# megvii-research/basedet

Hardware: AMD Instinct MI355X
Metric: images/sec training RetinaNet-R50-FPN 1333x800 (higher is better)
Workload: dtype bf16; 1 GPU; retinanet_r50_800x1344 train step (fwd+bwd+allreduce+SGD), DummyLoader boxes, random-init weights, inputs resident in HBM; per_gpu_batch=16, global_batch=16, parallelism=dp1

## Files before the change

### basedet_amd/_lib.py

```python
import ctypes as C
import os

import torch

_HERE = os.path.dirname(os.path.abspath(__file__))
LIB_PATH = os.environ.get("BASEDET_HIP_LIB") or os.path.join(_HERE, "lib", "libbasedet_hip.so")

BD_MAX_SEGS = 8
ABI_VERSION = 112
EPI_RELU, EPI_ADD_BEFORE, EPI_ADD_AFTER, EPI_MASK, EPI_SPARSE = 1, 2, 4, 8, 16


class BasedetHipError(RuntimeError):
    pass


class ConvDesc(C.Structure):
    _fields_ = [
        ("N", C.c_int32), ("Cin", C.c_int32), ("Cout", C.c_int32), ("R", C.c_int32), ("S", C.c_int32),
        ("stride", C.c_int32), ("pad", C.c_int32), ("nseg", C.c_int32),
        ("Hi", C.c_int32 * BD_MAX_SEGS), ("Wi", C.c_int32 * BD_MAX_SEGS),
        ("Ho", C.c_int32 * BD_MAX_SEGS), ("Wo", C.c_int32 * BD_MAX_SEGS),
        ("in_off", C.c_int32 * BD_MAX_SEGS), ("out_off", C.c_int32 * BD_MAX_SEGS),
        ("in_pix_per_img", C.c_int32), ("out_pix_per_img", C.c_int32),
        ("route", C.c_int32 * 4), ("sr_seed", C.c_uint32),
        ("gskip", C.c_int32), ("gskip_ws", C.c_void_p), ("gskip_ws_bytes", C.c_size_t),
        ("gskip_gmap", C.c_void_p), ("gskip_gmap_bytes", C.c_size_t), ("gskip_dxmap", C.c_void_p), ("gskip_dxmap_bytes", C.c_size_t),
        ("gskip_dx_clean", C.c_int32),
        ("fwd_map", C.c_void_p), ("fwd_map_bytes", C.c_size_t), ("fwd_clean", C.c_int32),
    ]


class PackDesc(C.Structure):
    _fields_ = [("w", C.c_void_p), ("row_scale", C.c_void_p), ("w_fwd", C.c_void_p), ("w_dgrad", C.c_void_p),
                ("Cout", C.c_int32), ("RS", C.c_int32), ("Cin", C.c_int32), ("block_start", C.c_int32)]


class ImageDesc(C.Structure):
    _fields_ = [("offset", C.c_int64), ("src_h", C.c_int32), ("src_w", C.c_int32), ("dst_h", C.c_int32), ("dst_w", C.c_int32),
                ("flip", C.c_int32), ("reserved_", C.c_int32 * 1)]


_P, _I, _L, _F, _Z = C.c_void_p, C.c_int, C.c_int64, C.c_float, C.c_size_t
_D = C.POINTER(ConvDesc)
# ... 223 lines not shown
```

### basedet_amd/csrc/conv3x3_pp.hip

```cpp
#include "conv3x3_pp128_body.h"

namespace {

constexpr int PH = 4, PW = 16, IH = PH + 2, IW = PW + 2;
constexpr int NPATCH = 4;
constexpr int XROWS = NPATCH * IH * IW;
constexpr int X_PITCH = 144;
constexpr int X_BYTES = XROWS * X_PITCH;
constexpr int XPASSES = 7;
constexpr int TILE_CO = 256;
constexpr int W_SLOT = TILE_CO * 128;
constexpr int NSLOT = 3;
constexpr int W_BYTES = NSLOT * W_SLOT;
constexpr int GTAB_TILES = 16;
constexpr int GTAB_BYTES = GTAB_TILES * NPATCH * 32;
constexpr int LDS_BYTES = W_BYTES + X_BYTES + TILE_CO * 4 + GTAB_BYTES;
constexpr int MAX_SEG = BD_MAX_SEGS;
constexpr int TAIL_CO = 64;

struct PSeg { int patch_start, H, W, pw, src_off, dst_off; float inv_pw; };

struct PParams {
    const bf16_raw* src;
    const bf16_raw* w;
// ... 696 lines not shown
        const int grid128 = cdiv(p.total_patches, NPATCH) * cdiv(p.CO, 128);
        if (!gn_part && g_patch_pp < 2 && 3 * cdiv(grid, 256) >= 2 * cdiv(grid128, 256)) return 1;
    }
    BD_ONCE_PER_DEVICE(
        (void)hipFuncSetAttribute(reinterpret_cast<const void*>(&conv3x3_pp_kernel<0>), hipFuncAttributeMaxDynamicSharedMemorySize, LDS_BYTES);
        (void)hipFuncSetAttribute(reinterpret_cast<const void*>(&conv3x3_pp_kernel<1>), hipFuncAttributeMaxDynamicSharedMemorySize, LDS_BYTES);
        (void)hipFuncSetAttribute(reinterpret_cast<const void*>(&conv3x3_pp_kernel<1, false, true>), hipFuncAttributeMaxDynamicSharedMemorySize,
                                  LDS_BYTES);
        (void)hipFuncSetAttribute(reinterpret_cast<const void*>(&conv3x3_pp_kernel<0, false, true>), hipFuncAttributeMaxDynamicSharedMemorySize,
                                  LDS_BYTES));
    bd_note_kernel("conv3x3_pp_kernel");
    if (sparse) {
        const int tot = p.total_patches;
        p.sp_keep_dead = in_place ? 1 : 0;
        p.sp_stride = tot;
        if (d->gskip_gmap) {
            BdGskipMap gm;
            bd_gskip_map_layout(d, 0, &gm);
            const int* m = (const int*)d->gskip_gmap;
            p.sp_hdr = m; p.sp_live = m + gm.live; p.sp_list = m + gm.list;
        } else {
            int* mk = (int*)d->gskip_ws;
            p.sp_live = mk + tot; p.sp_list = mk + 2 * tot; p.sp_count = mk + 3 * tot;
            bd_gskip_scan(d, src, PH, PW, mk, stream);
            bd_gskip_compact(d, PH, PW, mk, mk + tot, mk + 2 * tot, mk + 3 * tot, stream);
        }
        if (d->gskip_dxmap) {
            BdGskipMap xm;
            bd_gskip_map_layout(d, 1, &xm);
            p.sp_ohdr = (int*)d->gskip_dxmap; p.sp_olist = p.sp_ohdr + xm.list;
// ... 72 lines not shown
```

### basedet_amd/csrc/conv_igemm.hip

```cpp
#include "igemm_params.h"

using namespace igemm;

namespace {

template <int BK>
struct Cfg {
    static constexpr int CHUNKS = BK / 8;
    static constexpr int ROWS_PER_PASS = 256 / CHUNKS;
    static constexpr int PASSES = 128 / ROWS_PER_PASS;
    static constexpr int LDS_STRIDE = BK == 64 ? 160 : 64;
    static constexpr int TILE_BYTES = 128 * LDS_STRIDE;
    __device__ static __forceinline__ int off(int row, int chunk) {
        if constexpr (BK == 64) return row * LDS_STRIDE + chunk * 16;
        else return row * 64 + ((chunk ^ ((row >> 1) & 3)) << 4);
    }
};

template <int BK, bool PRE, bool BUF>
__global__ __launch_bounds__(256) void conv_igemm_kernel(const IgemmParams p) {
    using C = Cfg<BK>;
    extern __shared__ __attribute__((aligned(16))) unsigned char smem[];
    unsigned char* tiles = smem;
    unsigned int* s_tapmask = reinterpret_cast<unsigned int*>(smem);
// ... 527 lines not shown
    BD_ROUTE(d);
    return conv2d_fwd_impl(d, x, w_packed, bias, add, y, ybits, y8, q_scale, flags, stream);
}

extern "C" int bd_conv2d_fwd_bits(const bd_conv_desc* d, const void* x, const void* w_packed, const float* bias, const void* add, void* y,
                                  uint32_t* ybits, int flags, bd_stream_t stream) {
    BD_ROUTE(d);
    BD_REQUIRE(ybits != nullptr, "conv2d_fwd_bits: null ybits");
    return conv2d_fwd_impl(d, x, w_packed, bias, add, y, ybits, nullptr, 1.f, flags, stream);
}

static int conv2d_dgrad_impl(const bd_conv_desc* d, const void* g, const void* w_packed_t, const void* add, const void* mask,
                             const unsigned* maskbits, void* dx, void* dx8, float q_scale, int flags, bd_stream_t stream) {
    if (int e = check_desc(d)) return e;
    BD_REQUIRE(g && w_packed_t && dx, "conv2d_dgrad: null pointer");
    if (d->gskip && is_3x3s1(d) && !d->gskip_gmap) {
        const size_t need = bd_conv2d_dgrad_gskip_bytes(d);
        BD_REQUIRE(d->gskip_ws && d->gskip_ws_bytes >= need, "conv2d_dgrad: gskip scratch %zu < required %zu bytes (or NULL)",
                   (size_t)d->gskip_ws_bytes, need);
    }
    if (d->gskip_gmap || d->gskip_dxmap || d->gskip_dx_clean) {
        BD_REQUIRE(d->gskip && is_3x3s1(d) && g_use_patch3x3 && !maskbits && !dx8 && bd_conv3x3_pp_maps_ok(d, flags, add, dx),
                   "conv2d_dgrad: liveness maps need gskip on a 3x3 / stride 1 / pad 1 descriptor into more than 128 channels with an overwriting "
                   "(or, without gskip_dxmap, in-place accumulating) epilogue on the default route");
        BD_REQUIRE(!d->gskip_gmap || d->gskip_gmap_bytes >= bd_conv2d_gskip_map_bytes(d, 0), "conv2d_dgrad: gskip_gmap %zu < required %zu bytes",
                   (size_t)d->gskip_gmap_bytes, bd_conv2d_gskip_map_bytes(d, 0));
        BD_REQUIRE(!d->gskip_dxmap || d->gskip_dxmap_bytes >= bd_conv2d_gskip_map_bytes(d, 1), "conv2d_dgrad: gskip_dxmap %zu < required %zu bytes",
                   (size_t)d->gskip_dxmap_bytes, bd_conv2d_gskip_map_bytes(d, 1));
        BD_REQUIRE(!d->gskip_dx_clean || d->gskip_dxmap, "conv2d_dgrad: gskip_dx_clean needs gskip_dxmap (the list the promise refers to)");
    }
    if (d->stride == 1) flags &= ~BD_EPI_SPARSE;
// ... 93 lines not shown
```

### basedet_amd/csrc/conv_wgrad.hip

```cpp
#include <vector>
#include "common.h"

namespace {

constexpr int TILE = 128;
constexpr int ROW_PITCH = 288;
constexpr int MAX_SEG = BD_MAX_SEGS;

struct WSeg {
    int m_start;
    int Ho, Wo, per_img;
    float inv_per_img, inv_wo;
    int Hi, Wi, in_off, out_off;
};

struct WgradParams {
    const bf16_raw* x;
    const bf16_raw* g;
    float* slab;
    int Cin, Cout, R, S, stride, pad;
    int M, nseg;
    int in_pix_per_img, out_pix_per_img;
    int ci_tiles, co_tiles, splits, steps_per_split, total_steps;
    WSeg seg[MAX_SEG];
// ... 285 lines not shown
    const int max_splits = pl.total_steps / 4 > 0 ? pl.total_steps / 4 : 1;
    if (splits > max_splits) splits = max_splits;
    pl.steps_per_split = cdiv(pl.total_steps, splits);
    pl.splits = cdiv(pl.total_steps, pl.steps_per_split);
    return pl;
}

}

int bd_wgrad1x1_splits(const bd_conv_desc* d);
int bd_wgrad1x1_launch(const bd_conv_desc* d, const void* x, const void* g, float* slab, int* splits_out, hipStream_t stream);
int bd_wgrad3x3_splits(const bd_conv_desc* d, int* total_patches_out, int* patches_per_img_out);
int bd_wgrad3x3_launch(const bd_conv_desc* d, const void* x, const void* g, float* slab, float* csum, int* splits_out, hipStream_t stream);
bool bd_wgrad3x3r_eligible(const bd_conv_desc* d);
size_t bd_wgrad3x3r_slab_bytes(const bd_conv_desc* d, int* splits_out);
int bd_wgrad3x3r_launch(const bd_conv_desc* d, const void* x, const void* g, float* slab, float* csum, const int* gflags, int* splits_out,
                        hipStream_t stream);
int bd_wgrad3x3r_gskip_patches(const bd_conv_desc* d);
void bd_gskip_scan(const bd_conv_desc* d, const void* g, int ph, int pw, int* mask, hipStream_t stream);
void bd_wgrad3x3r_entry(const bd_conv_desc* d, BdRedEntry* e);
bool bd_wgrad1x1r_eligible(const bd_conv_desc* d);
size_t bd_wgrad1x1r_slab_bytes(const bd_conv_desc* d, int* splits_out);
int bd_wgrad1x1r_launch(const bd_conv_desc* d, const void* x, const void* g, float* slab, int* splits_out, hipStream_t stream);
void bd_wgrad1x1r_entry(const bd_conv_desc* d, BdRedEntry* e);

int bd_route_wgrad(int use_tr) {
    g_wgrad_use_tr = use_tr & 1;
    g_wgrad_use_3x3 = (use_tr & 2) ? 0 : 1;
    g_wgrad_use_ring = (use_tr & 4) ? 0 : 1;
    if (!(use_tr & 1)) g_wgrad_use_3x3 = 0;
    return BD_OK;
}
// ... 154 lines not shown
        BdRedEntry es[2] = {we, {}};
        int n = 1;
        if (dbias && fused_csum) es[n++] = plain_entry((const float*)extra, splits, d->Cout, 1, nullptr, dbias, accumulate);
        if (q) {
            for (int k = 0; k < n; ++k) q->entries.push_back(es[k]);
        } else {
            launch_batch(es, n, (hipStream_t)stream);
            BD_CHECK_LAUNCH("bd_conv2d_wgrad(reduce)");
        }
        return (dbias && !fused_csum) ? bias_fallback() : BD_OK;
    };
    if (g_wgrad_use_3x3 && g_wgrad_use_ring && bd_wgrad3x3r_eligible(d)) {
        int splitsr = 1;
        bd_note_kernel("conv_wgrad3x3_ring_kernel");
        int* gflags = nullptr;
        if (gskip_patches(d) > 0) {
            if (d->gskip_gmap) {
                BdGskipMap gm;
                bd_gskip_map_layout(d, 0, &gm);
                BD_REQUIRE(d->gskip_gmap_bytes >= gm.ints * sizeof(int) && gm.p8 == gskip_patches(d),
                           "conv2d_wgrad: gskip_gmap %zu < required %zu bytes", (size_t)d->gskip_gmap_bytes, gm.ints * sizeof(int));
                gflags = (int*)d->gskip_gmap + gm.m8;
            } else {
                gflags = (int*)((unsigned char*)ws + align256(wgrad_ws_base(d)));
                bd_gskip_scan(d, g, 8, 8, gflags, (hipStream_t)stream);
            }
        }
        bd_wgrad3x3r_launch(d, x, g, (float*)ws, dbias ? (float*)extra : nullptr, gflags, &splitsr, (hipStream_t)stream);
        BD_CHECK_LAUNCH("bd_conv2d_wgrad(3x3 ring)");
        BdRedEntry e{};
        bd_wgrad3x3r_entry(d, &e);
        e.slab = (const float*)ws; e.splits = splitsr; e.row_scale = row_scale; e.dw = dw; e.accumulate = accumulate;
        return finish(e, splitsr, true);
    }
    if (g_wgrad_use_3x3 && is_3x3s1(d)) {
        int splits3 = 1;
        bd_note_kernel("conv_wgrad3x3_kernel");
        bd_wgrad3x3_launch(d, x, g, (float*)ws, dbias ? (float*)extra : nullptr, &splits3, (hipStream_t)stream);
        BD_CHECK_LAUNCH("bd_conv2d_wgrad(3x3)");
        return finish(plain_entry((const float*)ws, splits3, (long long)d->Cout * 9 * d->Cin, 9 * d->Cin, row_scale, dw, accumulate), splits3, true);
    }
    if (g_wgrad_use_3x3 && g_wgrad_use_ring && bd_wgrad1x1r_eligible(d)) {
        int splitsr = 1;
// ... 48 lines not shown
```

### basedet_amd/csrc/conv_wgrad3x3_ring.hip

```cpp
#include <stdlib.h>
#include "common.h"
#include "wgrad_reduce.h"

namespace {

constexpr int RK_CI = 64, RK_CO = 128;
constexpr int XW = 10;
constexpr int X_PIECES = 13;
constexpr int X_BYTES = X_PIECES * 1024;
constexpr int G_PIECES = 16;
constexpr int G_BYTES = G_PIECES * 1024;
constexpr int STAGE = X_BYTES + G_BYTES;
constexpr int DEPTH = 3;
constexpr int NSTAGE = 5;
constexpr int LDS_BYTES = NSTAGE * STAGE;
constexpr int REGS = 36;
constexpr unsigned X_NONE = 0x80000000u;
constexpr int LIST_MAX = 3072;

typedef __attribute__((address_space(3))) void lds_void_rk_t;

struct RSeg { int patch_start, H, W, pw, in_off, out_off, Hi, Wi; };

struct RParams {
    const bf16_raw* x;
    const bf16_raw* g;
    float* slab;
    float* csum;
    const int* gflags;
    int Cin, Cout, N, nseg;
    int in_ppi, out_ppi;
    unsigned x_bytes, g_bytes;
    int patches_per_img, total_patches, patches_per_split;
    int ci_tiles, co_tiles;
    RSeg seg[BD_MAX_SEGS];
};

#ifdef BD_RK_STAMP
__device__ unsigned long long g_rk_stamp[8][8];
#endif

#ifndef BD_RK_ABLATE
#define BD_RK_ABLATE 0
#endif
__device__ unsigned long long g_rk_clk[2];

__device__ __forceinline__ void rk_dma16(__amdgpu_buffer_rsrc_t rsrc, unsigned lds_addr, unsigned voff, int soff = 0) {
    asm volatile("s_mov_b32 m0, %1\n\ts_nop 0\n\tbuffer_load_dwordx4 %0, %2, %3 offen lds" : : "v"(voff), "s"(lds_addr), "s"(rsrc), "s"(soff) : "memory");
}

// ... 13 lines not shown
    const int tiles = p.ci_tiles * p.co_tiles;
    const int split = bid / tiles;
    bid -= split * tiles;
    const int ci_tile = bid / p.co_tiles, co_tile = bid - ci_tile * p.co_tiles;
    const int ci0 = ci_tile * RK_CI, co0 = co_tile * RK_CO;
    const int pbeg = split * p.patches_per_split;
    int pend = pbeg + p.patches_per_split;
    if (pend > p.total_patches) pend = p.total_patches;
    int nsteps = pend > pbeg ? pend - pbeg : 0;
    int* live_list = reinterpret_cast<int*>(smem + LDS_BYTES);
    if constexpr (SPARSE) {
        __shared__ int wsum[8];
        int base = 0;
        for (int c0 = 0; c0 < nsteps; c0 += 512) {
            const int i = c0 + tid;
            const bool lv = i < nsteps && p.gflags[pbeg + i] != 0;
            const unsigned long long bal = __ballot(lv);
            const int pre = __popcll(bal & ((1ull << lane) - 1ull));
            if (lane == 0) wsum[wave] = __popcll(bal);
            __syncthreads();
            int off = base, tot = 0;
#pragma unroll
            for (int w = 0; w < 8; ++w) {
                off += w < wave ? wsum[w] : 0;
                tot += wsum[w];
            }
            if (lv) live_list[off + pre] = i;
            base += tot;
            __syncthreads();
        }
        nsteps = base;
// ... 312 lines not shown
        if (d->Hi[s] != d->Ho[s] || d->Wi[s] != d->Wo[s]) return false;
    return true;
}

size_t bd_wgrad3x3r_slab_bytes(const bd_conv_desc* d, int* splits_out) {
    const RPlan pl = ring_plan(d);
    if (splits_out) *splits_out = pl.splits;
    return (size_t)pl.splits * pl.tiles * 8 * REGS * 1024;
}

int bd_wgrad3x3r_gskip_patches(const bd_conv_desc* d) {
    const RPlan pl = ring_plan(d);
    return pl.per <= LIST_MAX ? pl.total : 0;
}

int bd_wgrad3x3r_launch(const bd_conv_desc* d, const void* x, const void* g, float* slab, float* csum, const int* gflags, int* splits_out,
                        hipStream_t stream) {
    RParams p{};
    const RPlan pl = ring_plan(d);
    p.gflags = gflags;
    p.x = (const bf16_raw*)x; p.g = (const bf16_raw*)g; p.slab = slab; p.csum = csum;
    p.Cin = d->Cin; p.Cout = d->Cout; p.N = d->N; p.nseg = d->nseg;
    p.in_ppi = d->in_pix_per_img; p.out_ppi = d->out_pix_per_img;
    p.x_bytes = (unsigned)((long long)d->N * d->in_pix_per_img * d->Cin * 2);
    p.g_bytes = (unsigned)((long long)d->N * d->out_pix_per_img * d->Cout * 2);
    p.total_patches = pl.total; p.patches_per_img = pl.ppi; p.patches_per_split = pl.per;
    p.ci_tiles = pl.ci_tiles; p.co_tiles = pl.co_tiles;
    int ps = 0;
    for (int s = 0; s < d->nseg; ++s) {
        RSeg& sg = p.seg[s];
        sg.patch_start = ps; sg.H = d->Ho[s]; sg.W = d->Wo[s]; sg.pw = cdiv(d->Wo[s], 8);
        sg.in_off = d->in_off[s]; sg.out_off = d->out_off[s]; sg.Hi = d->Hi[s]; sg.Wi = d->Wi[s];
        ps += cdiv(d->Ho[s], 8) * sg.pw;
    }
    BD_ONCE_PER_DEVICE(
        (void)hipFuncSetAttribute(reinterpret_cast<const void*>(&conv_wgrad3x3_ring_kernel<false>), hipFuncAttributeMaxDynamicSharedMemorySize,
                                  LDS_BYTES);
        (void)hipFuncSetAttribute(reinterpret_cast<const void*>(&conv_wgrad3x3_ring_kernel<true>), hipFuncAttributeMaxDynamicSharedMemorySize,
                                  LDS_BYTES + LIST_MAX * 4));
    if (gflags && pl.per <= LIST_MAX)
        hipLaunchKernelGGL(conv_wgrad3x3_ring_kernel<true>, dim3(pl.splits * pl.tiles), dim3(512), LDS_BYTES + LIST_MAX * 4, stream, p);
    else
        hipLaunchKernelGGL(conv_wgrad3x3_ring_kernel<false>, dim3(pl.splits * pl.tiles), dim3(512), LDS_BYTES, stream, p);
    *splits_out = pl.splits;
    return 0;
}

void bd_wgrad3x3r_entry(const bd_conv_desc* d, BdRedEntry* e) {
    const RPlan pl = ring_plan(d);
    e->kind = 1; e->regs = REGS; e->co_tiles = pl.co_tiles; e->tci = RK_CI; e->tco = RK_CO; e->fi = 0; e->fj = 0;
    e->Cin = d->Cin; e->Cout = d->Cout; e->n4 = 8 * REGS * 64 * pl.tiles; e->row_len = 0;
}
```

### basedet_amd/csrc/image_ops.hip

```cpp
#include <stdarg.h>

#include <cmath>
#include "common.h"

static thread_local std::string g_bd_error = "";
int bd_num_cus() {
    static std::mutex mu;
    static int cached[256] = {0};
    int dev = 0;
    if (hipGetDevice(&dev) != hipSuccess || dev < 0 || dev > 255) return 256;
    std::lock_guard<std::mutex> g(mu);
    if (!cached[dev]) {
        int n = 0;
        cached[dev] = (hipDeviceGetAttribute(&n, hipDeviceAttributeMultiprocessorCount, dev) == hipSuccess && n > 0) ? n : 256;
    }
    return cached[dev];
}

void bd_set_error(const char* fmt, ...) {
    char buf[512];
    va_list ap;
    va_start(ap, fmt);
    vsnprintf(buf, sizeof(buf), fmt, ap);
    va_end(ap);
    g_bd_error = buf;
}
extern "C" const char* bd_last_error_string(void) { return g_bd_error.c_str(); }
static thread_local const char* g_bd_last_kernel = "";
void bd_note_kernel(const char* name) { g_bd_last_kernel = name; }
extern "C" const char* bd_conv_last_kernel(void) { return g_bd_last_kernel; }
extern "C" int bd_version(void) { return 112; }

namespace {

constexpr int HALO_Y = 3, HALO_X = 4;

__global__ void pad_normalize_kernel(const float* __restrict__ in, int N, int H, int W, int Hp, int Wp,
                                     float m0, float m1, float m2, float s0, float s1, float s2,
                                     bf16_raw* __restrict__ out) {
    const int Hb = Hp + 2 * HALO_Y, Wb = Wp + 2 * HALO_X;
    const long long total = (long long)N * Hb * Wb;
    for (long long i = (long long)blockIdx.x * blockDim.x + threadIdx.x; i < total; i += (long long)gridDim.x * blockDim.x) {
        const int xb = (int)(i % Wb);
        const long long t = i / Wb;
        const int yb = (int)(t % Hb);
        const int n = (int)(t / Hb);
// ... 574 lines not shown
```

### basedet_amd/models/engine.py

```python
import numpy as np
import torch

from .. import ops
from ..ops import Geom

BN_EPS = 1e-5


class ParamArena:

    def __init__(self, device):
        self.device = device
        self.entries = []
        self.total = 0
        self.w = self.g = self.v = None

    def reserve(self, name, shape):
        n = int(np.prod(shape))
        off = self.total
        self.entries.append((name, tuple(shape), off, n))
        self.total += (n + 63) // 64 * 64
        return len(self.entries) - 1

    def allocate(self):
# ... 13 lines not shown
        self.name, self.cin, self.cout_real, self.k, self.stride, self.pad = name, cin, cout, k, stride, pad
        self.norm = norm
        self.cout = cout_pad or cout
        self.bn_prefix, self.has_bias, self.trainable = bn_prefix, has_bias, trainable
        self.device = device
        self.w = self.b = self.gw = self.gb = None
        self.row_scale = None
        self.w_fwd = torch.empty((self.cout, k * k, cin), dtype=torch.bfloat16, device=device)
        self.w_dgrad = torch.empty((cin, k * k, self.cout), dtype=torch.bfloat16, device=device) if trainable else None
        self._desc_cache = {}
        self.gskip = False
        self._gskip_cache = {}
        self._gskip_ws = None
        self._chain = (None, None, False)
        self._chain_cache = {}
        self._fwd_map_cache = {}
        self.fp8 = False
        self.fp8_dgrad = False
        self.fp8_wgrad = False
        self.fp8_1x1 = False
        self.fp8_1x1_dgrad = False
        self.w_q8 = self.w_scale8 = self.w_q8t = self.w_scale8t = None
        self.act_scale = 1.0
        self.grad_scale = 4096.0
        self.amax_slot = None
        self.probe_ctl = None
        self.q8_scratch = None

    def bind(self, arena, params):
        w = torch.from_numpy(params[self.name + ".weight"]).permute(0, 2, 3, 1).contiguous()
# ... 94 lines not shown
            d = ops.conv_desc(gin, gout, self.cin, self.cout, self.k, self.k, self.stride, self.pad)
            self._desc_cache[key] = d
        return d

    def bwd_desc(self, gin: Geom, gout: Geom):
        d = self.desc(gin, gout)
        if not self.gskip:
            return d
        h = self._gskip_cache.get(id(d))
        if h is None:
            n = (max(ops.conv2d_dgrad_gskip_bytes(d), 4) + 3) // 4
            if self._gskip_ws is None or self._gskip_ws.numel() < n:
                self._gskip_ws = torch.empty(n, dtype=torch.int32, device=self.device)
                self._gskip_cache.clear()
            h = self._gskip_cache[id(d)] = (ops.gskip_desc(d, self._gskip_ws), d)
        gmap, dxmap, clean = self._chain
        if gmap is None and dxmap is None:
            return h[0]
        key = (id(d), self._gskip_ws.data_ptr(), gmap.data_ptr() if gmap is not None else 0, dxmap.data_ptr() if dxmap is not None else 0, clean)
        c = self._chain_cache.get(key)
        if c is None:
            if len(self._chain_cache) > 64:
                self._chain_cache.clear()
            c = self._chain_cache[key] = (ops.gskip_desc(d, self._gskip_ws, gmap=gmap, dxmap=dxmap, dx_clean=clean), d)
        return c[0]

    def set_chain(self, gmap=None, dxmap=None, dx_clean=False):
        self._chain = (gmap, dxmap, bool(dx_clean) and dxmap is not None) if self.gskip else (None, None, False)

    def fwd_map_desc(self, gin: Geom, gout: Geom, fmap, clean):
        d = self.desc(gin, gout)
        key = (id(d), fmap.data_ptr(), bool(clean))
        c = self._fwd_map_cache.get(key)
        if c is None:
            if len(self._fwd_map_cache) > 64:
                self._fwd_map_cache.clear()
            c = self._fwd_map_cache[key] = (ops.fwd_map_desc(d, fmap, clean), d)
        return c[0]

    def forward(self, x, gin, gout, y, add=None, relu=False, bits=None, x8=None, y8=None, q_scale=1.0, fwd_map=None, fwd_clean=False):
        flags = (ops.EPI_RELU if relu else 0) | (ops.EPI_ADD_BEFORE if add is not None else 0)
        if fwd_map is not None:
            assert not self.fp8 and not self.fp8_1x1 and bits is None and y8 is None
# ... 263 lines not shown
```

### basedet_amd/models/retinanet.py

```python
import torch

from .. import ops
from ..streams import fork, join
from ..utils.registry import registers
from . import params as P
from .engine import PaddedClsConv
from .fpn_base import FPNDetector, _round_up


@registers.models.register()
class RetinaNet(FPNDetector):
    READS_MATCHER = True

    @staticmethod
    def init_params(cfg, seed=0):
        return P.init_retinanet_params(cfg, seed)

    @classmethod
    def check_config(cls, cfg):
        super().check_config(cfg)
        cls.check_anchor_config(cfg, matcher=cls.READS_MATCHER)
        if not cfg.MODEL.HEAD.get("WITH_NORM", True):
            raise ValueError("MODEL.HEAD.WITH_NORM = False is not supported for the RetinaNet family: only True (the default) is implemented")

# ... 3 lines not shown
        self.num_anchors = len(m.ANCHOR.SCALES[0]) * len(m.ANCHOR.RATIOS[0])
        nc = m.HEAD.NUM_CONVS
        self.cls_tower = [add(f"head.cls_subnet.{2 * i}", ch, ch, 3, 1, 1, bias=True) for i in range(nc)]
        self.box_tower = [add(f"head.bbox_subnet.{2 * i}", ch, ch, 3, 1, 1, bias=True) for i in range(nc)]
        A, K = self.num_anchors, self.num_classes
        self.cls_score = self.convs["head.cls_score"] = PaddedClsConv("head.cls_score", ch, A, K, 3, 1, 1, self.device)
        self.cls_ld = self.cls_score.cls_ld
        self.box_ld = _round_up(A * 4, 8)
        self.bbox_pred = add("head.bbox_pred", ch, A * 4, 3, 1, 1, bias=True, cout_pad=self.box_ld)
        if bool(m.get("SPARSE_BOX_BWD", True)) and m.get("WEIGHT_DTYPE", "bf16") == "bf16":
            for c in self.box_tower + [self.bbox_pred]:
                c.gskip = True
        self.sparse_chain = bool(m.get("SPARSE_BOX_CHAIN", True))
        self.sparse_box_fwd = (bool(m.get("SPARSE_BOX_FWD", True)) and type(self) is RetinaNet and nc >= 1 and nc <= 8
                               and all(c.gskip for c in self.box_tower + [self.bbox_pred]))
        self._build_base_anchors()

    def _head_convs(self):
        return self.cls_tower + self.box_tower + [self.cls_score, self.bbox_pred]

    def _plan_head(self, pl):
        ch = self.fpn_ch
        N = pl.N
        C = pl._carve
        bf = torch.bfloat16

        def act(g, c):
            return C.empty((g.pixels, c), bf)

        nc = len(self.cls_tower)
# ... 4 lines not shown
        pl.offsets = act(pl.pyr, self.box_ld)
        pl.d_logits = C.like(pl.logits)
        pl.d_offsets = C.like(pl.offsets)
        pl.g_tower = [[act(pl.pyr, ch) for _ in range(nc)] for _ in range(2)]
        pl.g_map = None
        if self.sparse_chain and all(c.gskip for c in self.box_tower + [self.bbox_pred]):
            nb = ops.conv2d_gskip_map_bytes(self.box_tower[0].desc(pl.pyr, pl.pyr))
            if nb:
                pl.g_map = [C.empty(((nb + 3) // 4,), torch.int32) for _ in range(nc)]
        pl.chain_epoch = None
        pl.f_map = None
        if self.sparse_box_fwd:
            nb = ops.fwd_live_map_bytes(self.box_tower[0].desc(pl.pyr, pl.pyr))
            if nb:
                pl.f_map = [C.empty(((nb + 3) // 4,), torch.int32) for _ in range(nc)]
        pl.fwd_epoch = None
        pl.fwd_skip = None
        pl.fwd_skipped = False
        tw = lambda: C.empty((pl.pyr.pixels, ch), torch.uint8)
        pl.cls_act8 = [tw() if c.fp8 else None for c in self.cls_tower]
        pl.box_act8 = [tw() if c.fp8 else None for c in self.box_tower]
        tg = self.fp8_grad_twins
        pl.g_tower8 = [[tw() if (c.fp8_dgrad and tg) else None for c in tower] for tower in (self.cls_tower, self.box_tower)]
        pl.g_P8 = tw() if (tg and all(t[0].fp8_dgrad for t in (self.cls_tower, self.box_tower))) else None
        self._plan_anchors(pl)
        tot = pl.A_total
        pl.labels = C.empty((N, tot), torch.int32)
        pl.match_idx = C.empty((N, tot), torch.int32)
        pl.gt_offsets = C.empty((N, tot, 4), torch.float32)
        pl.num_fg = C.zeros((1,), torch.int32)
# ... 29 lines not shown
        pl = pre["plan"]
        self._cur = pl
        m = self.cfg.MODEL
        gt = pre["gt_boxes"]
        num_gt = pre["img_info"][:, 4].to(torch.int32).contiguous()
        N, Gmax = gt.shape[0], gt.shape[1]
        ws = self._scratch("assign", N * Gmax * 4).view(torch.float32)
        thr = m.MATCHER.THRESHOLDS
        side = self.streams.aux() if m.get("ASSIGN_ON_SIDE_STREAM", True) else None
        with fork(side):
            ops.retina_assign_encode(pl.anchors, gt, num_gt, thr[0], thr[1], m.MATCHER.ALLOW_LOW_QUALITY, m.BOX_REG.MEAN,
                                     m.BOX_REG.STD, pl.labels, pl.match_idx, pl.gt_offsets, pl.num_fg, ws)
            if pl.f_map is not None and self.streams.aux() is not None:
                clean = pl.fwd_epoch == self.plan_arena.epoch
                pl.fwd_epoch = self.plan_arena.epoch
                ops.fwd_live_maps(self.box_tower[0].desc(pl.pyr, pl.pyr), pl.labels, self.num_anchors, pl.f_map[::-1], reset=not clean)
                pl.fwd_skip = (clean,)
        self.network_forward(pl)
        join(side)
        pl.loss_buf.zero_()
        rows = N * pl.A_total
        ops.focal_loss_fwd_bwd(pl.logits, pl.labels, rows, self.num_classes, m.LOSSES.FOCAL_LOSS_ALPHA,
                               m.LOSSES.FOCAL_LOSS_GAMMA, pl.num_fg, 1.0, pl.loss_buf[0:1], pl.d_logits, ld=self.cls_ld)
        ops.smooth_l1_fwd_bwd(pl.offsets, pl.gt_offsets, pl.labels, pl.pyr.pixels, self.num_anchors, self.box_ld,
                              m.LOSSES.SMOOTH_L1_BETA, pl.num_fg, m.LOSSES.REG_LOSS_WEIGHT, pl.loss_buf[1:2], pl.d_offsets)
        cls_loss, reg_loss = pl.loss_buf[0], pl.loss_buf[1]
        return {"total_loss": cls_loss + reg_loss, "cls_loss": cls_loss, "reg_loss": reg_loss}

    def head_backward(self, pl, ws, cws):
        pyr = pl.pyr
        for ti, (tower, acts, pred, dpred) in enumerate(((self.cls_tower, pl.cls_act, self.cls_score, pl.d_logits),
                                                         (self.box_tower, pl.box_act, self.bbox_pred, pl.d_offsets))):
            gbuf, g8 = pl.g_tower[ti], pl.g_tower8[ti]
            n = len(tower)
            maps = pl.g_map if (ti == 1 and self.sparse_chain and all(c.gskip for c in tower + [pred])) else None
            if ti == 1:
                clean = maps is not None and pl.chain_epoch == self.plan_arena.epoch
                pl.chain_epoch = self.plan_arena.epoch if maps is not None else None
                if maps is not None:
                    pred.set_chain(None, maps[n - 1], clean)
                    for i in range(n):
                        tower[i].set_chain(maps[i], maps[i - 1] if i > 0 else None, clean)
            gs = tower[n - 1].grad_scale
            self._wgrad(pred, acts[-1], dpred, pyr, pyr, ws, cws)
            tw = g8[n - 1] if pred.dgrad_writes_twin(pyr, pyr) else None
            if not pred.dgrad(dpred, pyr, pyr, gbuf[n - 1], mask=acts[-1], dx8=tw, q_scale=gs):
                tw = None
            act8 = pl.cls_act8 if ti == 0 else pl.box_act8
            for i in range(n - 1, -1, -1):
                x = acts[i - 1] if i > 0 else pl.P
                x8 = (act8[i - 1] if i > 0 else pl.P8) if tw is not None else None
                self._wgrad(tower[i], x, gbuf[i], pyr, pyr, ws, cws, x8=x8, g8=tw)
                if i > 0:
                    nxt = g8[i - 1] if tower[i].dgrad_writes_twin(pyr, pyr) else None
                    wrote = tower[i].dgrad(gbuf[i], pyr, pyr, gbuf[i - 1], mask=acts[i - 1], g8=tw, dx8=nxt, q_scale=tower[i - 1].grad_scale)
                    tw = nxt if wrote else None
                else:
                    wrote_p = tower[i].dgrad(gbuf[i], pyr, pyr, pl.g_P, first=(ti == 0), g8=tw,
                                             dx8=pl.g_P8 if tower[i].dgrad_writes_twin(pyr, pyr) else None,
                                             q_scale=self.output[self.fpn_stages[0]].grad_scale)
        for c in self.box_tower + [self.bbox_pred]:
            c.set_chain()
        pl.g_P8_ready = pl.g_P8 is not None and bool(wrote_p)

    def _debug_head(self, pl, out, lvl):
        if getattr(pl, "fwd_skipped", False):
            t = pl.P
            for c, a in zip(self.box_tower, pl.box_act):
                c.forward(t, pl.pyr, pl.pyr, a, relu=True); t = a
            self.bbox_pred.forward(t, pl.pyr, pl.pyr, pl.offsets)
            pl.fwd_skipped = False
            pl.fwd_epoch = None
        for i in range(pl.pyr.nlev):
            for k in range(len(self.cls_tower)):
                out[f"cls{k}_{i}"] = lvl(pl.cls_act[k], i)
                out[f"box{k}_{i}"] = lvl(pl.box_act[k], i)
            lg = lvl(pl.logits, i)
# ... 13 lines not shown
```

### basedet_amd/ops.py

```python
import ctypes as C
from dataclasses import dataclass, field
from typing import List, Optional

import torch

from . import _lib
from ._lib import ConvDesc, EPI_ADD_AFTER, EPI_ADD_BEFORE, EPI_MASK, EPI_RELU, EPI_SPARSE, check, f32arr, i32arr, ptr, stream_ptr


@dataclass
class Geom:
    N: int
    H: List[int]
    W: List[int]
    off: List[int] = field(default_factory=list)
    pix_per_img: int = 0

    def __post_init__(self):
        if not self.off:
            o = 0
            self.off = []
            for h, w in zip(self.H, self.W):
                self.off.append(o)
                o += h * w
# ... 87 lines not shown

def conv2d_dgrad_gskip_bytes(d):
    return int(L().bd_conv2d_dgrad_gskip_bytes(C.byref(d)))


def conv2d_gskip_map_bytes(d, of_dx=False):
    return int(L().bd_conv2d_gskip_map_bytes(C.byref(d), int(bool(of_dx))))


def gskip_map_scan(d, t, gmap, of_dx=False):
    check(L().bd_gskip_map_scan(C.byref(d), int(bool(of_dx)), ptr(t), ptr(gmap), gmap.numel() * gmap.element_size(), stream_ptr()),
          "bd_gskip_map_scan")
    return gmap


def gskip_desc(d, scratch=None, gmap=None, dxmap=None, dx_clean=False):
    h = ConvDesc.from_buffer_copy(d)
    h.gskip = 1
    if scratch is not None:
        h.gskip_ws = scratch.data_ptr()
        h.gskip_ws_bytes = scratch.numel() * scratch.element_size()
    if gmap is not None:
        h.gskip_gmap = gmap.data_ptr()
        h.gskip_gmap_bytes = gmap.numel() * gmap.element_size()
    if dxmap is not None:
        h.gskip_dxmap = dxmap.data_ptr()
        h.gskip_dxmap_bytes = dxmap.numel() * dxmap.element_size()
    h.gskip_dx_clean = int(bool(dx_clean))
    return h


def fwd_live_map_bytes(d):
    return int(L().bd_fwd_live_map_bytes(C.byref(d)))


def fwd_live_maps(d, labels, A, maps, reset=False):
    if labels.dtype != torch.int32 or labels.numel() != d.N * d.out_pix_per_img * A:
        raise _lib.BasedetHipError(f"fwd_live_maps: labels must be int32 with N * pixels * A = {d.N * d.out_pix_per_img * A} entries")
    nb = min(m.numel() * m.element_size() for m in maps)
    arr = (C.c_void_p * len(maps))(*[ptr(m).value for m in maps])
    check(L().bd_fwd_live_maps(C.byref(d), ptr(labels), int(A), len(maps), arr, nb, int(bool(reset)), stream_ptr()), "bd_fwd_live_maps")
    return maps

# ... 806 lines not shown
```

### include/basedet_hip.h

```cpp
#ifndef BASEDET_HIP_H
#define BASEDET_HIP_H

#include <stddef.h>
#include <stdint.h>

#ifdef __cplusplus
extern "C" {
#endif

#define BD_OK 0
#define BD_EINVAL (-1)
#define BD_ELAUNCH (-2)
#define BD_EWORKSPACE (-3)

#define BD_MAX_SEGS 8

#define BD_EPI_RELU 1
#define BD_EPI_ADD_BEFORE 2
#define BD_EPI_ADD_AFTER 4
#define BD_EPI_MASK 8
#define BD_EPI_SPARSE 16

typedef void* bd_stream_t;

// ... 8 lines not shown
    int32_t in_off[BD_MAX_SEGS], out_off[BD_MAX_SEGS];
    int32_t in_pix_per_img, out_pix_per_img;
    int32_t route[4];
    uint32_t sr_seed;
    int32_t gskip;
    void* gskip_ws;
    size_t gskip_ws_bytes;
    void* gskip_gmap;
    size_t gskip_gmap_bytes;
    void* gskip_dxmap;
    size_t gskip_dxmap_bytes;
    int32_t gskip_dx_clean;
    void* fwd_map;
    size_t fwd_map_bytes;
    int32_t fwd_clean;
} bd_conv_desc;

const char* bd_last_error_string(void);
int bd_version(void);
const char* bd_conv_last_kernel(void);
int bd_probe_mfma_rate(double seconds, double* tflops_out, double* clock_mhz_out, bd_stream_t stream);

int bd_probe_kernel_clock(const char* kernel, int reset, double* clock_mhz_out, double* busy_ms_out);


int bd_conv2d_fwd(const bd_conv_desc* d, const void* x, const void* w_packed, const float* bias,
                  const void* add, void* y, int flags, bd_stream_t stream);

int bd_conv2d_dgrad(const bd_conv_desc* d, const void* g, const void* w_packed_t, const void* add,
                    const void* mask, void* dx, int flags, bd_stream_t stream);
// ... 402 lines not shown
```

Baseline: 725.1 images/sec.

## Reuse forward live-patch maps to drive sparse box-tower dgrad and wgrad

The label-derived forward live maps, plus an extra map for the tower input, now drive sparsity in the box-tower backward pass. This replaces the separate gradient scans or chain maps. The 3x3 patch dgrad kernel reads the forward map as both input and output live lists. The wgrad ring kernel translates its 8x8 patch ids into the 4x16 forward-map granularity to decide liveness. This removes the per-layer gskip scan and compaction launches in backward, at the cost of coarser or over-approximate liveness and more descriptor and ABI fields.

```diff
diff --git a/basedet_amd/_lib.py b/basedet_amd/_lib.py
--- a/basedet_amd/_lib.py
+++ b/basedet_amd/_lib.py
@@ -7,7 +7,7 @@
 LIB_PATH = os.environ.get("BASEDET_HIP_LIB") or os.path.join(_HERE, "lib", "libbasedet_hip.so")
 
 BD_MAX_SEGS = 8
-ABI_VERSION = 112
+ABI_VERSION = 113
 EPI_RELU, EPI_ADD_BEFORE, EPI_ADD_AFTER, EPI_MASK, EPI_SPARSE = 1, 2, 4, 8, 16
 
 
@@ -28,6 +28,8 @@
         ("gskip_gmap", C.c_void_p), ("gskip_gmap_bytes", C.c_size_t), ("gskip_dxmap", C.c_void_p), ("gskip_dxmap_bytes", C.c_size_t),
         ("gskip_dx_clean", C.c_int32),
         ("fwd_map", C.c_void_p), ("fwd_map_bytes", C.c_size_t), ("fwd_clean", C.c_int32),
+        ("gskip_dx_fmap", C.c_void_p), ("gskip_dx_fmap_bytes", C.c_size_t), ("gskip_dx_fclean", C.c_int32),
+        ("gskip_g_fmap", C.c_void_p), ("gskip_g_fmap_bytes", C.c_size_t),
     ]
 
 
diff --git a/basedet_amd/csrc/conv3x3_pp.hip b/basedet_amd/csrc/conv3x3_pp.hip
--- a/basedet_amd/csrc/conv3x3_pp.hip
+++ b/basedet_amd/csrc/conv3x3_pp.hip
@@ -734,6 +734,16 @@
         const int tot = p.total_patches;
         p.sp_keep_dead = in_place ? 1 : 0;
         p.sp_stride = tot;
+        if (d->gskip_dx_fmap) {
+            BdFwdMap fm;
+            bd_fwd_map_layout(d, &fm);
+            int* m = (int*)d->gskip_dx_fmap;
+            p.sp_hdr = m; p.sp_live = m + fm.live; p.sp_list = m + fm.list;
+            p.sp_ohdr = m; p.sp_olist = m + fm.list; p.sp_oflip = 1;
+            p.sp_clean = d->gskip_dx_fclean ? 1 : 0;
+            hipLaunchKernelGGL((conv3x3_pp_kernel<1, false, true>), dim3(p.main_grid), dim3(512), LDS_BYTES, stream, p);
+            return 0;
+        }
         if (d->gskip_gmap) {
             BdGskipMap gm;
             bd_gskip_map_layout(d, 0, &gm);
diff --git a/basedet_amd/csrc/conv_igemm.hip b/basedet_amd/csrc/conv_igemm.hip
--- a/basedet_amd/csrc/conv_igemm.hip
+++ b/basedet_amd/csrc/conv_igemm.hip
@@ -565,7 +565,16 @@
                              const unsigned* maskbits, void* dx, void* dx8, float q_scale, int flags, bd_stream_t stream) {
     if (int e = check_desc(d)) return e;
     BD_REQUIRE(g && w_packed_t && dx, "conv2d_dgrad: null pointer");
-    if (d->gskip && is_3x3s1(d) && !d->gskip_gmap) {
+    if (d->gskip_dx_fmap || d->gskip_dx_fclean) {
+        BD_REQUIRE(d->gskip_dx_fmap && !d->gskip_gmap && !d->gskip_dxmap && !d->gskip_dx_clean,
+                   "conv2d_dgrad: gskip_dx_fmap stands alone (no gskip_gmap / gskip_dxmap / gskip_dx_clean), and gskip_dx_fclean needs it");
+        BD_REQUIRE(d->gskip && is_3x3s1(d) && g_use_patch3x3 && !maskbits && !dx8 && bd_conv3x3_pp_maps_ok(d, flags, add, dx),
+                   "conv2d_dgrad: gskip_dx_fmap needs gskip on a 3x3 / stride 1 / pad 1 descriptor into more than 128 channels with an overwriting "
+                   "or in-place accumulating epilogue on the default route");
+        BD_REQUIRE(d->gskip_dx_fmap_bytes >= bd_fwd_live_map_bytes(d), "conv2d_dgrad: gskip_dx_fmap %zu < required %zu bytes",
+                   (size_t)d->gskip_dx_fmap_bytes, bd_fwd_live_map_bytes(d));
+    }
+    if (d->gskip && is_3x3s1(d) && !d->gskip_gmap && !d->gskip_dx_fmap) {
         const size_t need = bd_conv2d_dgrad_gskip_bytes(d);
         BD_REQUIRE(d->gskip_ws && d->gskip_ws_bytes >= need, "conv2d_dgrad: gskip scratch %zu < required %zu bytes (or NULL)",
                    (size_t)d->gskip_ws_bytes, need);
diff --git a/basedet_amd/csrc/conv_wgrad.hip b/basedet_amd/csrc/conv_wgrad.hip
--- a/basedet_amd/csrc/conv_wgrad.hip
+++ b/basedet_amd/csrc/conv_wgrad.hip
@@ -323,8 +323,8 @@
 int bd_wgrad3x3_launch(const bd_conv_desc* d, const void* x, const void* g, float* slab, float* csum, int* splits_out, hipStream_t stream);
 bool bd_wgrad3x3r_eligible(const bd_conv_desc* d);
 size_t bd_wgrad3x3r_slab_bytes(const bd_conv_desc* d, int* splits_out);
-int bd_wgrad3x3r_launch(const bd_conv_desc* d, const void* x, const void* g, float* slab, float* csum, const int* gflags, int* splits_out,
-                        hipStream_t stream);
+int bd_wgrad3x3r_launch(const bd_conv_desc* d, const void* x, const void* g, float* slab, float* csum, const int* gflags, const int* fflags,
+                        int* splits_out, hipStream_t stream);
 int bd_wgrad3x3r_gskip_patches(const bd_conv_desc* d);
 void bd_gskip_scan(const bd_conv_desc* d, const void* g, int ph, int pw, int* mask, hipStream_t stream);
 void bd_wgrad3x3r_entry(const bd_conv_desc* d, BdRedEntry* e);
@@ -509,7 +509,15 @@
         int splitsr = 1;
         bd_note_kernel("conv_wgrad3x3_ring_kernel");
         int* gflags = nullptr;
-        if (gskip_patches(d) > 0) {
+        const int* fflags = nullptr;
+        if (d->gskip_g_fmap) {
+            BdFwdMap fm;
+            bd_fwd_map_layout(d, &fm);
+            BD_REQUIRE(d->gskip && !d->gskip_gmap, "conv2d_wgrad: gskip_g_fmap needs gskip and stands instead of gskip_gmap");
+            BD_REQUIRE(d->gskip_g_fmap_bytes >= fm.ints * sizeof(int), "conv2d_wgrad: gskip_g_fmap %zu < required %zu bytes",
+                       (size_t)d->gskip_g_fmap_bytes, fm.ints * sizeof(int));
+            if (gskip_patches(d) > 0) fflags = (const int*)d->gskip_g_fmap + fm.live;
+        } else if (gskip_patches(d) > 0) {
             if (d->gskip_gmap) {
                 BdGskipMap gm;
                 bd_gskip_map_layout(d, 0, &gm);
@@ -521,7 +529,7 @@
                 bd_gskip_scan(d, g, 8, 8, gflags, (hipStream_t)stream);
             }
         }
-        bd_wgrad3x3r_launch(d, x, g, (float*)ws, dbias ? (float*)extra : nullptr, gflags, &splitsr, (hipStream_t)stream);
+        bd_wgrad3x3r_launch(d, x, g, (float*)ws, dbias ? (float*)extra : nullptr, gflags, fflags, &splitsr, (hipStream_t)stream);
         BD_CHECK_LAUNCH("bd_conv2d_wgrad(3x3 ring)");
         BdRedEntry e{};
         bd_wgrad3x3r_entry(d, &e);
diff --git a/basedet_amd/csrc/conv_wgrad3x3_ring.hip b/basedet_amd/csrc/conv_wgrad3x3_ring.hip
--- a/basedet_amd/csrc/conv_wgrad3x3_ring.hip
+++ b/basedet_amd/csrc/conv_wgrad3x3_ring.hip
@@ -34,6 +34,9 @@
     int patches_per_img, total_patches, patches_per_split;
     int ci_tiles, co_tiles;
     RSeg seg[BD_MAX_SEGS];
+    const int* fflags;
+    int f4_ppi;
+    int f4_start[BD_MAX_SEGS];
 };
 
 #ifdef BD_RK_STAMP
@@ -77,7 +80,23 @@
         int base = 0;
         for (int c0 = 0; c0 < nsteps; c0 += 512) {
             const int i = c0 + tid;
-            const bool lv = i < nsteps && p.gflags[pbeg + i] != 0;
+            bool lv = false;
+            if (i < nsteps) {
+                if (p.fflags) {
+                    const int pid = pbeg + i;
+                    const int n = pid / p.patches_per_img, rem = pid - n * p.patches_per_img;
+                    int s = 0;
+#pragma unroll
+                    for (int k = 1; k < BD_MAX_SEGS; ++k)
+                        if (k < p.nseg && rem >= p.seg[k].patch_start) s = k;
+                    const int local = rem - p.seg[s].patch_start, by = local / p.seg[s].pw, bx = local - by * p.seg[s].pw;
+                    const int rows4 = (p.seg[s].H + 3) >> 2, pw16 = (p.seg[s].W + 15) >> 4;
+                    const int* f = p.fflags + (long long)n * p.f4_ppi + p.f4_start[s] + 2 * by * pw16 + (bx >> 1);
+                    lv = f[0] != 0 || (2 * by + 1 < rows4 && f[pw16] != 0);
+                } else {
+                    lv = p.gflags[pbeg + i] != 0;
+                }
+            }
             const unsigned long long bal = __ballot(lv);
             const int pre = __popcll(bal & ((1ull << lane) - 1ull));
             if (lane == 0) wsum[wave] = __popcll(bal);
@@ -420,11 +439,12 @@
     return pl.per <= LIST_MAX ? pl.total : 0;
 }
 
-int bd_wgrad3x3r_launch(const bd_conv_desc* d, const void* x, const void* g, float* slab, float* csum, const int* gflags, int* splits_out,
-                        hipStream_t stream) {
+int bd_wgrad3x3r_launch(const bd_conv_desc* d, const void* x, const void* g, float* slab, float* csum, const int* gflags, const int* fflags,
+                        int* splits_out, hipStream_t stream) {
     RParams p{};
     const RPlan pl = ring_plan(d);
     p.gflags = gflags;
+    p.fflags = fflags;
     p.x = (const bf16_raw*)x; p.g = (const bf16_raw*)g; p.slab = slab; p.csum = csum;
     p.Cin = d->Cin; p.Cout = d->Cout; p.N = d->N; p.nseg = d->nseg;
     p.in_ppi = d->in_pix_per_img; p.out_ppi = d->out_pix_per_img;
@@ -439,12 +459,17 @@
         sg.in_off = d->in_off[s]; sg.out_off = d->out_off[s]; sg.Hi = d->Hi[s]; sg.Wi = d->Wi[s];
         ps += cdiv(d->Ho[s], 8) * sg.pw;
     }
+    {
+        int p4 = 0;
+        for (int s = 0; s < d->nseg; ++s) { p.f4_start[s] = p4; p4 += cdiv(d->Ho[s], 4) * cdiv(d->Wo[s], 16); }
+        p.f4_ppi = p4;
+    }
     BD_ONCE_PER_DEVICE(
         (void)hipFuncSetAttribute(reinterpret_cast<const void*>(&conv_wgrad3x3_ring_kernel<false>), hipFuncAttributeMaxDynamicSharedMemorySize,
                                   LDS_BYTES);
         (void)hipFuncSetAttribute(reinterpret_cast<const void*>(&conv_wgrad3x3_ring_kernel<true>), hipFuncAttributeMaxDynamicSharedMemorySize,
                                   LDS_BYTES + LIST_MAX * 4));
-    if (gflags && pl.per <= LIST_MAX)
+    if ((gflags || fflags) && pl.per <= LIST_MAX)
         hipLaunchKernelGGL(conv_wgrad3x3_ring_kernel<true>, dim3(pl.splits * pl.tiles), dim3(512), LDS_BYTES + LIST_MAX * 4, stream, p);
     else
         hipLaunchKernelGGL(conv_wgrad3x3_ring_kernel<false>, dim3(pl.splits * pl.tiles), dim3(512), LDS_BYTES, stream, p);
diff --git a/basedet_amd/csrc/image_ops.hip b/basedet_amd/csrc/image_ops.hip
--- a/basedet_amd/csrc/image_ops.hip
+++ b/basedet_amd/csrc/image_ops.hip
@@ -29,7 +29,7 @@
 static thread_local const char* g_bd_last_kernel = "";
 void bd_note_kernel(const char* name) { g_bd_last_kernel = name; }
 extern "C" const char* bd_conv_last_kernel(void) { return g_bd_last_kernel; }
-extern "C" int bd_version(void) { return 112; }
+extern "C" int bd_version(void) { return 113; }
 
 namespace {
 
diff --git a/basedet_amd/models/engine.py b/basedet_amd/models/engine.py
--- a/basedet_amd/models/engine.py
+++ b/basedet_amd/models/engine.py
@@ -51,6 +51,7 @@
         self._gskip_ws = None
         self._chain = (None, None, False)
         self._chain_cache = {}
+        self._fmaps = (None, False, None)
         self._fwd_map_cache = {}
         self.fp8 = False
         self.fp8_dgrad = False
@@ -175,6 +176,15 @@
                 self._gskip_ws = torch.empty(n, dtype=torch.int32, device=self.device)
                 self._gskip_cache.clear()
             h = self._gskip_cache[id(d)] = (ops.gskip_desc(d, self._gskip_ws), d)
+        dx_fmap, dx_fclean, g_fmap = self._fmaps
+        if dx_fmap is not None or g_fmap is not None:
+            key = (id(d), "f", dx_fmap.data_ptr() if dx_fmap is not None else 0, dx_fclean, g_fmap.data_ptr() if g_fmap is not None else 0)
+            c = self._chain_cache.get(key)
+            if c is None:
+                if len(self._chain_cache) > 64:
+                    self._chain_cache.clear()
+                c = self._chain_cache[key] = (ops.gskip_desc(d, dx_fmap=dx_fmap, dx_fclean=dx_fclean, g_fmap=g_fmap), d)
+            return c[0]
         gmap, dxmap, clean = self._chain
         if gmap is None and dxmap is None:
             return h[0]
@@ -188,6 +198,9 @@
 
     def set_chain(self, gmap=None, dxmap=None, dx_clean=False):
         self._chain = (gmap, dxmap, bool(dx_clean) and dxmap is not None) if self.gskip else (None, None, False)
+
+    def set_fmaps(self, dx_fmap=None, dx_fclean=False, g_fmap=None):
+        self._fmaps = (dx_fmap, bool(dx_fclean) and dx_fmap is not None, g_fmap) if self.gskip else (None, False, None)
 
     def fwd_map_desc(self, gin: Geom, gout: Geom, fmap, clean):
         d = self.desc(gin, gout)
diff --git a/basedet_amd/models/retinanet.py b/basedet_amd/models/retinanet.py
--- a/basedet_amd/models/retinanet.py
+++ b/basedet_amd/models/retinanet.py
@@ -41,6 +41,7 @@
         self.sparse_chain = bool(m.get("SPARSE_BOX_CHAIN", True))
         self.sparse_box_fwd = (bool(m.get("SPARSE_BOX_FWD", True)) and type(self) is RetinaNet and nc >= 1 and nc <= 8
                                and all(c.gskip for c in self.box_tower + [self.bbox_pred]))
+        self.sparse_box_bwd_maps = bool(m.get("SPARSE_BOX_BWD_MAPS", True)) and self.sparse_box_fwd and nc + 1 <= 8
         self._build_base_anchors()
 
     def _head_convs(self):
@@ -75,6 +76,8 @@
             nb = ops.fwd_live_map_bytes(self.box_tower[0].desc(pl.pyr, pl.pyr))
             if nb:
                 pl.f_map = [C.empty(((nb + 3) // 4,), torch.int32) for _ in range(nc)]
+        pl.f_map_p = C.empty((pl.f_map[0].numel(),), torch.int32) if (self.sparse_box_bwd_maps and pl.f_map is not None) else None
+        pl.fmap_gen, pl.fmap_kept, pl.bwd_gen = 0, False, None
         pl.fwd_epoch = None
         pl.fwd_skip = None
         pl.fwd_skipped = False
@@ -134,7 +137,9 @@
             if pl.f_map is not None and self.streams.aux() is not None:
                 clean = pl.fwd_epoch == self.plan_arena.epoch
                 pl.fwd_epoch = self.plan_arena.epoch
-                ops.fwd_live_maps(self.box_tower[0].desc(pl.pyr, pl.pyr), pl.labels, self.num_anchors, pl.f_map[::-1], reset=not clean)
+                maps = pl.f_map[::-1] + ([pl.f_map_p] if pl.f_map_p is not None else [])
+                ops.fwd_live_maps(self.box_tower[0].desc(pl.pyr, pl.pyr), pl.labels, self.num_anchors, maps, reset=not clean)
+                pl.fmap_gen, pl.fmap_kept = pl.fmap_gen + 1, clean
                 pl.fwd_skip = (clean,)
         self.network_forward(pl)
         join(side)
@@ -154,9 +159,19 @@
             gbuf, g8 = pl.g_tower[ti], pl.g_tower8[ti]
             n = len(tower)
             maps = pl.g_map if (ti == 1 and self.sparse_chain and all(c.gskip for c in tower + [pred])) else None
+            fmaps = (ti == 1 and self.sparse_box_bwd_maps and pl.f_map_p is not None and pl.fwd_skipped
+                     and all(c.gskip for c in tower + [pred]))
             if ti == 1:
-                clean = maps is not None and pl.chain_epoch == self.plan_arena.epoch
-                pl.chain_epoch = self.plan_arena.epoch if maps is not None else None
+                by_maps = pl.bwd_gen is not None
+                fclean = fmaps and by_maps and pl.fmap_kept and pl.bwd_gen == pl.fmap_gen - 1 and pl.chain_epoch == self.plan_arena.epoch
+                pl.bwd_gen = pl.fmap_gen if fmaps else None
+                if fmaps:
+                    maps = None
+                    pred.set_fmaps(pl.f_map[n - 1], fclean, None)
+                    for i in range(n):
+                        tower[i].set_fmaps(pl.f_map[i - 1] if i > 0 else pl.f_map_p, fclean and i > 0, pl.f_map[i])
+                clean = maps is not None and not by_maps and pl.chain_epoch == self.plan_arena.epoch
+                pl.chain_epoch = self.plan_arena.epoch if (maps is not None or fmaps) else None
                 if maps is not None:
                     pred.set_chain(None, maps[n - 1], clean)
                     for i in range(n):
@@ -181,6 +196,7 @@
                                              q_scale=self.output[self.fpn_stages[0]].grad_scale)
         for c in self.box_tower + [self.bbox_pred]:
             c.set_chain()
+            c.set_fmaps()
         pl.g_P8_ready = pl.g_P8 is not None and bool(wrote_p)
 
     def _debug_head(self, pl, out, lvl):
diff --git a/basedet_amd/ops.py b/basedet_amd/ops.py
--- a/basedet_amd/ops.py
+++ b/basedet_amd/ops.py
@@ -125,7 +125,7 @@
     return gmap
 
 
-def gskip_desc(d, scratch=None, gmap=None, dxmap=None, dx_clean=False):
+def gskip_desc(d, scratch=None, gmap=None, dxmap=None, dx_clean=False, dx_fmap=None, dx_fclean=False, g_fmap=None):
     h = ConvDesc.from_buffer_copy(d)
     h.gskip = 1
     if scratch is not None:
@@ -138,6 +138,13 @@
         h.gskip_dxmap = dxmap.data_ptr()
         h.gskip_dxmap_bytes = dxmap.numel() * dxmap.element_size()
     h.gskip_dx_clean = int(bool(dx_clean))
+    if dx_fmap is not None:
+        h.gskip_dx_fmap = dx_fmap.data_ptr()
+        h.gskip_dx_fmap_bytes = dx_fmap.numel() * dx_fmap.element_size()
+    h.gskip_dx_fclean = int(bool(dx_fclean))
+    if g_fmap is not None:
+        h.gskip_g_fmap = g_fmap.data_ptr()
+        h.gskip_g_fmap_bytes = g_fmap.numel() * g_fmap.element_size()
     return h
 
 
diff --git a/include/basedet_hip.h b/include/basedet_hip.h
--- a/include/basedet_hip.h
+++ b/include/basedet_hip.h
@@ -46,6 +46,11 @@
     void* fwd_map;
     size_t fwd_map_bytes;
     int32_t fwd_clean;
+    void* gskip_dx_fmap;
+    size_t gskip_dx_fmap_bytes;
+    int32_t gskip_dx_fclean;
+    void* gskip_g_fmap;
+    size_t gskip_g_fmap_bytes;
 } bd_conv_desc;
 
 const char* bd_last_error_string(void);
```

Measured after the change: 729.3 images/sec, median of 6. Within noise of the previous version (+0.6%).
